# ru-wang/slam-plus-plus

Measured on AMD Instinct MI355X. Metric: Λ-solve block-nnz/sec + batch GN iters/sec, Venice BA, 1→8 MI355X, higher is better.
Workload: dtype f64; 1 GPU; venice871-shaped synthetic BA (871 cams, 530304 points, 2838740 observations, LM-damped); nnzb=3369915, n=1596138, mode=schur+dense, n_reduced=5226, schur_pairs=12875640, parallelism=single GPU

## Files before the change

### include/spp_hip.h

```cpp
#ifndef SPP_HIP_H
#define SPP_HIP_H

#include <stddef.h>
#include <stdint.h>

#ifdef __cplusplus
extern "C" {
#endif

#define SPP_OK            0
#define SPP_NOT_POSDEF    1
#define SPP_E_BADARG     -1
#define SPP_E_NOMEM      -2
#define SPP_E_HIP        -3
#define SPP_E_NO_DEVICE  -4
#define SPP_E_STATE      -5
#define SPP_E_UNSUPPORTED -6

#define SPP_MODE_AUTO     0
#define SPP_MODE_SPARSE   1
#define SPP_MODE_SCHUR    2
#define SPP_MODE_SCHUR_SPARSE 3

#define SPP_FLAG_PROFILE  1
// ... 153 lines not shown
#define SPP_PHASE_BACKSUBST 6
#define SPP_PHASE_ASSEMBLE  7
#define SPP_PHASE_TOTAL     8
#define SPP_N_PHASES        9
int spp_get_phase_ms(spp_ctx *ctx, double *ms_out );
int spp_get_dominant_kernel(spp_ctx *ctx, double *ms_total, int64_t *n_launches, double *flops);

int spp_microbench_copy(spp_ctx *ctx, size_t bytes, int iters, double *gb_per_s);
int spp_microbench_mfma_f64(spp_ctx *ctx, int iters, double *tflops);
int spp_microbench_ctile(spp_ctx *ctx, int n, int iters, double *gb_per_s);
int spp_microbench_update(spp_ctx *ctx, int64_t m, int iters, double *ms_per_launch);

int spp_dense_potrf_upper(spp_ctx *ctx, double *d_A, int64_t n, int64_t ld);
int spp_dense_posv(spp_ctx *ctx, double *d_A, int64_t n, int64_t ld, double *d_b);
int spp_dense_posv_masked(spp_ctx *ctx, double *d_A, int64_t n, int64_t ld, double *d_b, const uint64_t *words, int64_t nwords);
int spp_tile_mask_host(int64_t n, int bs, int64_t nblk, const int32_t *i1, const int32_t *i2, int has_rhs, int fill,
	uint64_t *words, int64_t *n_updates);
int spp_schur_tile_mask_host(int64_t nb, const int32_t *dim, const int64_t *col_ptr, const int64_t *row_idx, int shard_rank,
	int shard_world, uint64_t *words);
int spp_schur_cam_order_host(int64_t nb, const int32_t *dim, const int64_t *col_ptr, const int64_t *row_idx, int shard_rank,
	int shard_world, int flags, const int64_t *order_in, int64_t *cam_order, double *figures);
int spp_tail_order_host(int64_t n, int has_rhs, const uint64_t *words, int64_t nwords, int resident, int early, double beta,
	int32_t *table, int32_t *info);
int spp_dense_gemm_tn_sub(spp_ctx *ctx, int64_t m, int64_t n, int64_t k,
	const double *d_A, int64_t lda, const double *d_B, int64_t ldb, double *d_C, int64_t ldc);
int spp_dense_gemm_tn_sub_upper(spp_ctx *ctx, int64_t m, int64_t n, int64_t k,
	const double *d_A, int64_t lda, const double *d_B, int64_t ldb, double *d_C, int64_t ldc);
int spp_dense_front_factor(spp_ctx *ctx, double *d_F, int64_t ld, int64_t w, int64_t h, double *d_image);

const char *spp_version(void);

#ifdef __cplusplus
}
#endif
#endif
```

### slam_plus_plus_amd/api.py

```python
import ctypes
import os

import numpy as np

_HERE = os.path.dirname(os.path.abspath(__file__))
LIB_PATH = os.environ.get("SPP_LIB") or os.path.join(_HERE, "libspp_hip.so")

SPP_OK, SPP_NOT_POSDEF = 0, 1
MODE_AUTO, MODE_SPARSE, MODE_SCHUR, MODE_SCHUR_SPARSE, MODE_SCHUR_MIS = 0, 1, 2, 3, 4
FLAG_PROFILE = 1
INFO = dict(MODE=0, N=1, NNZB=2, NVALS=3, FACTOR_NNZ=4, FACTOR_FLOPS=5, N_REDUCED=6, N_POSES=7,
            N_LANDMARKS=8, SCHUR_PAIRS=9, N_OBS=10, SOLVE_BYTES=11, N_SUPERNODES=12, N_LEVELS=13, S_LD=14, S_NNZB=15, DENSE_STREAMED=16,
            LM_STREAM=17, BS_GROUPS=18, SCHUR_SIDE=19, S_CLEAR=20, S_DEVICE_PTR=21, ASM_HUB_CHUNK=22)
PHASES = ["permute", "schur_inv", "schur_gemm", "schur_rhs", "factor", "trisolve", "backsubst", "assemble", "total"]

EXPORTS = [
    "spp_create", "spp_destroy", "spp_free_memory", "spp_last_error", "spp_host_staging", "spp_set_stream", "spp_synchronize",
    "spp_analyze", "spp_set_shard", "spp_get_info", "spp_get_ordering", "spp_sparse_fronts", "spp_factor_solve",
    "spp_factor_solve_device", "spp_schur_buffer_size", "spp_schur_form", "spp_schur_finish",
    "spp_schur_packed_size", "spp_schur_pack", "spp_schur_unpack",
    "spp_assemble_analyze", "spp_assemble_get_structure", "spp_assemble_device", "spp_assemble_set_edge_weights",
    "spp_assemble_analyze_groups", "spp_assemble_groups_device", "spp_assemble_set_group_edge_weights",
    "spp_assemble_analyze_ternary", "spp_assemble_ternary_device", "spp_ba_intrinsics_linearize_device",
    "spp_ba_intrinsics_update_device",
    "spp_se2_linearize_at_device", "spp_se2_rb_linearize_device", "spp_slam2d_update_device",
    "spp_se3_linearize_at_device", "spp_se3_xyz_linearize_device", "spp_slam3d_update_device", "spp_rocv_range_linearize_device",
    "spp_rocv_cv_linearize_device", "spp_device_malloc",
    "spp_device_free", "spp_memcpy_h2d", "spp_memcpy_d2h", "spp_memcpy_d2d", "spp_get_phase_ms", "spp_get_dominant_kernel",
    "spp_microbench_copy", "spp_microbench_mfma_f64", "spp_microbench_ctile", "spp_microbench_update", "spp_block_ordering", "spp_schur_plan_host", "spp_set_profiling", "spp_se2_linearize_device", "spp_se2_update_device", "spp_ba_linearize_device", "spp_ba_stereo_linearize_device", "spp_ba_update_device", "spp_se3_linearize_device", "spp_se3_update_device", "spp_edge_chi2_device", "spp_edge_robust_weights_device", "spp_edge_hessian_maxdiag_device",
    "spp_lm_gain_denominator_device", "spp_dense_potrf_upper", "spp_dense_posv",
    "spp_dense_posv_masked", "spp_tile_mask_host", "spp_schur_tile_mask_host", "spp_tail_order_host", "spp_schur_cam_order_host",
    "spp_dense_gemm_tn_sub", "spp_dense_gemm_tn_sub_upper", "spp_dense_front_factor", "spp_version",
]

_lib = None
_c_i64p = ctypes.POINTER(ctypes.c_int64)
_c_i32p = ctypes.POINTER(ctypes.c_int32)
_c_f64p = ctypes.POINTER(ctypes.c_double)


class SppError(RuntimeError):
    """std::runtime_error of the C++ adapter (reference LinearSolver_Schur_GPU.cpp:734-797)."""


def load_library():
    global _lib
    if _lib is not None:
        return _lib
    if not os.path.exists(LIB_PATH):
        raise SppError("libspp_hip.so is not built: run `python -m slam_plus_plus_amd.build` "
                       "(hipcc --offload-arch=gfx950); there is no CPU fallback")
    lib = ctypes.CDLL(LIB_PATH)
    vp, i64, i32, dbl, cint = ctypes.c_void_p, ctypes.c_int64, ctypes.c_int32, ctypes.c_double, ctypes.c_int
    sig = {
# ... 47 lines not shown
        "spp_microbench_mfma_f64": (cint, [vp, cint, _c_f64p]),
        "spp_microbench_ctile": (cint, [vp, cint, cint, _c_f64p]),
        "spp_microbench_update": (cint, [vp, ctypes.c_int64, cint, _c_f64p]),
        "spp_block_ordering": (cint, [ctypes.c_int64, vp, vp, cint, vp]),
        "spp_schur_plan_host": (cint, [ctypes.c_int64, vp, vp, vp, cint, cint, cint, vp, vp]),
        "spp_set_profiling": (cint, [vp, cint]),
        "spp_se2_linearize_device": (cint, [vp, ctypes.c_int64, vp, vp, vp, vp, vp, vp, vp]),
        "spp_se2_update_device": (cint, [vp, ctypes.c_int64, vp, vp, cint, _c_f64p]),
        "spp_se3_linearize_device": (cint, [vp, ctypes.c_int64, vp, vp, vp, vp, vp, vp, vp]),
        "spp_se3_update_device": (cint, [vp, ctypes.c_int64, vp, vp, cint, _c_f64p]),
        "spp_edge_chi2_device": (cint, [vp, ctypes.c_int64, cint, vp, vp, _c_f64p]),
        "spp_edge_robust_weights_device": (cint, [vp, ctypes.c_int64, cint, cint, dbl, dbl, vp, vp]),
        "spp_edge_hessian_maxdiag_device": (cint, [vp, ctypes.c_int64, cint, cint, cint, vp, vp, vp, _c_f64p]),
        "spp_lm_gain_denominator_device": (cint, [vp, ctypes.c_int64, vp, vp, ctypes.c_double, _c_f64p]),
        "spp_ba_linearize_device": (cint, [vp, ctypes.c_int64, vp, vp, vp, vp, vp, vp, vp, vp, vp]),
        "spp_ba_stereo_linearize_device": (cint, [vp, ctypes.c_int64, vp, vp, vp, vp, vp, vp, vp, vp, vp]),
        "spp_ba_update_device": (cint, [vp, ctypes.c_int64, vp, vp, ctypes.c_int64, vp, vp, vp, ctypes.c_int64, cint, _c_f64p]),
        "spp_dense_potrf_upper": (cint, [vp, vp, i64, i64]),
        "spp_dense_posv": (cint, [vp, vp, i64, i64, vp]),
        "spp_dense_posv_masked": (cint, [vp, vp, i64, i64, vp, vp, i64]),
        "spp_tile_mask_host": (cint, [i64, cint, i64, vp, vp, cint, cint, vp, vp]),
        "spp_schur_tile_mask_host": (cint, [i64, vp, vp, vp, cint, cint, vp]),
        "spp_tail_order_host": (cint, [i64, cint, vp, i64, cint, cint, dbl, vp, vp]),
        "spp_schur_cam_order_host": (cint, [i64, vp, vp, vp, cint, cint, cint, vp, vp, vp]),
        "spp_dense_gemm_tn_sub": (cint, [vp, i64, i64, i64, vp, i64, vp, i64, vp, i64]),
        "spp_dense_gemm_tn_sub_upper": (cint, [vp, i64, i64, i64, vp, i64, vp, i64, vp, i64]),
        "spp_dense_front_factor": (cint, [vp, vp, i64, i64, i64, vp]),
        "spp_version": (ctypes.c_char_p, []),
    }
    for name, (res, args) in sig.items():
        fn = getattr(lib, name)
        fn.restype = res
        fn.argtypes = args
    _lib = lib
    return lib


def _ptr(a):
    return a.ctypes.data_as(ctypes.c_void_p)


ORDER_AMD, ORDER_ND = 0, 1


def block_ordering(lam, method=ORDER_AMD):
    lib = load_library()
# ... 56 lines not shown
    nc = int((dim == dim.max()).sum()) if not mis else int(dim.size)
    out = np.full(max(nc, 1), -1, dtype=np.int64)
    fig = np.zeros(8, dtype=np.float64)
    oin = None if order is None else np.ascontiguousarray(order, dtype=np.int64)
    if oin is not None and oin.size != nc:
        raise SppError("schur_cam_order_host: order must list every camera once")
    code = lib.spp_schur_cam_order_host(lam.nb, _ptr(dim), _ptr(col_ptr), _ptr(row_idx), shard_rank, shard_world,
                                        (1 if sparse_S else 0) | (2 if mis else 0),
                                        _ptr(oin) if oin is not None else None, _ptr(out), _ptr(fig))
    if code < 0:
        raise SppError("spp_schur_cam_order_host failed: %d" % code)
    keys = ("tiles", "updates", "path", "cost_us")
    natural = dict(zip(keys, (int(fig[0]), int(fig[1]), int(fig[2]), float(fig[3]))))
    chosen = dict(zip(keys, (int(fig[4]), int(fig[5]), int(fig[6]), float(fig[7]))))
    return out[out >= 0], bool(code), natural, chosen


def tail_order_host(n, words, has_rhs=True, resident=256, early=True, beta=0.0):
    lib = load_library()
    words = np.ascontiguousarray(words if words is not None else [], dtype=np.uint64)
    table = np.zeros(64 * 65 // 2 + 64, dtype=np.int32)
    info = np.zeros(5, dtype=np.int32)
    code = lib.spp_tail_order_host(int(n), 1 if has_rhs else 0, _ptr(words) if words.size else None, words.size, int(resident),
                                   1 if early else 0, float(beta), _ptr(table), _ptr(info))
    if code < 0:
        raise SppError("spp_tail_order_host failed: %d" % code)
    tiles = [(int(t) >> 16, int(t) & 0xffff) for t in table[:code]]
    return tiles, dict(zip(("n_early", "r_star", "rows_resident", "live_demand", "widest"), (int(v) for v in info)))


class DeviceArray:

    def __init__(self, ctx, n, dtype=np.float64):
        self.ctx, self.n, self.dtype = ctx, int(n), np.dtype(dtype)
        p = ctypes.c_void_p()
        ctx._check(ctx.lib.spp_device_malloc(ctx.h, self.n * self.dtype.itemsize, ctypes.byref(p)))
        self.ptr = p.value

    @classmethod
    def from_host(cls, ctx, arr):
        arr = np.ascontiguousarray(arr)
        d = cls(ctx, arr.size, arr.dtype)
        d.upload(arr)
        return d

    def upload(self, arr):
        arr = np.ascontiguousarray(arr, dtype=self.dtype)
        assert arr.size == self.n
        self.ctx._check(self.ctx.lib.spp_memcpy_h2d(self.ctx.h, self.ptr, _ptr(arr), arr.nbytes))

    def download(self):
# ... 347 lines not shown
```

### slam_plus_plus_amd/csrc/spp_api.cpp

```cpp

#include "spp_internal.h"
#include <string.h>
#include <new>

using namespace spp;

namespace spp {

void phases_reset(spp_ctx *ctx)
{
	if(!(ctx->flags & SPP_FLAG_PROFILE))
		return;
	if(!ctx->timer.created) {
		for(int i = 0; i < 2 * SPP_N_PHASES; ++ i)
			SPP_HIP_CHECK(hipEventCreate(&ctx->timer.ev[i]));
		ctx->timer.created = true;
	}
	for(int i = 0; i < SPP_N_PHASES; ++ i) {
		ctx->timer.used[i] = false;
		ctx->phase_ms[i] = 0;
	}
	ctx->dom_used = 0;
	ctx->dom_flops = 0;
}
// ... 1164 lines not shown
			*n_updates = upd;
		for(size_t q = 0; q < w.size(); ++ q)
			words[q] = w[q];
		return (int)w.size();
	} catch(...) {
		return SPP_E_NOMEM;
	}
}

int spp_tail_order_host(int64_t n, int has_rhs, const uint64_t *words, int64_t nwords, int resident, int early, double beta,
	int32_t *table, int32_t *info)
{
	const int64_t Tr = (n + DENSE_NB - 1) / DENSE_NB, Tc = has_rhs ? n / DENSE_NB + 1 : Tr;
	if(n <= 0 || Tr > 64 || Tc > 64 || nwords < 0 || (nwords && (!words || nwords != Tr)) || !table || !(beta >= 0))
		return SPP_E_BADARG;
	try {
		std::vector<uint64_t> bits((size_t)Tr + 1);
		const uint64_t all_cols = Tc == 64 ? ~0ull : (1ull << Tc) - 1;
		bits[0] = all_cols;
		for(int64_t i = 0; i < Tr; ++ i)
			bits[(size_t)i + 1] = (((nwords ? words[i] : all_cols) | (1ull << i)) & ~((1ull << i) - 1)) & all_cols;
		std::vector<int> order;
		int oinfo[5];
		const bool use = nwords && early;
		tail_order_table(bits, (int)Tr, (int)Tc, false, beta, use ? resident : 0, use, order, oinfo);
		for(size_t q = 0; q < order.size(); ++ q)
			table[q] = order[q];
		if(info)
			for(int q = 0; q < 5; ++ q)
				info[q] = oinfo[q];
		return (int)order.size();
	} catch(...) {
		return SPP_E_NOMEM;
	}
}

int spp_dense_posv_masked(spp_ctx *ctx, double *d_A, int64_t n, int64_t ld, double *d_b, const uint64_t *words, int64_t nwords)
{
	if(!ctx || !d_A || !d_b || n <= 0 || ld < n || nwords < 0 || (nwords && !words))
		return SPP_E_BADARG;
	SPP_TRY(ctx)
	SPP_HIP_CHECK(hipSetDevice(ctx->device));
	std::vector<uint64_t> mask(words, words + nwords);
	if(nwords) {
		SPP_REQUIRE(nwords == (n + DENSE_NB - 1) / DENSE_NB, SPP_E_BADARG, "posv: one mask word per tile row of 128");
		tile_mask_close(n, true, true, mask);
	}
	TileMaskGuard guard(ctx->dense, &mask);
	const int64_t ldp = ((n + 1 + DENSE_NB - 1) / DENSE_NB) * DENSE_NB;
	DevBuf<double> tmp;
	tmp.reserve((size_t)ldp * ldp);
	SPP_HIP_CHECK(hipMemsetAsync(tmp.p, 0, (size_t)ldp * ldp * sizeof(double), ctx->stream));
	SPP_HIP_CHECK(hipMemcpy2DAsync(tmp.p, ldp * sizeof(double), d_A, ld * sizeof(double), n * sizeof(double), n,
		hipMemcpyDeviceToDevice, ctx->stream));
// ... 55 lines not shown
```

### slam_plus_plus_amd/csrc/spp_dense.hip

```cpp

#include "spp_internal.h"
#include "spp_tiles.h"
#include "spp_dense_dev.h"
#include <stdio.h>
#include <stdlib.h>
#include <string.h>
#include <algorithm>
#include <vector>
#include <mutex>

namespace spp {


constexpr int BK = 16;
constexpr int LDS_STRIDE = 18;

template <int BM, int BN, int WM, int WN, int MODE, int DEPTH, int BKT, int SC1 = 0>
__device__ __forceinline__ void gemm_tn_tile(const int64_t m0, const int64_t n0, int64_t M, int64_t N, int K,
	const double *__restrict__ A, int64_t lda, const double *B, int64_t ldb, double *C, int64_t ldc, double *gemm_lds)
{
	constexpr int NWM = BM / WM, NWN = BN / WN, NT = NWM * NWN * 64;
	constexpr int TA = WM / 16, TB = WN / 16;
	constexpr int PPC = BKT / 2, LSTR = BKT + 2;
	constexpr int PA = (BM * PPC) / NT, PB = (BN * PPC) / NT;
// ... 1257 lines not shown
	for(int i = -1; i < Tr; ++ i) {
		const int64_t g = k + 1 + i;
		uint64_t w = (mask && g >= 0) ? ((*mask)[(size_t)g] >> (k + 1)) : all_cols;
		if(i >= 0)
			w = (w | (1ull << i)) & ~((1ull << i) - 1);
		bits[(size_t)i + 1] = w & all_cols;
	}
	hipStream_t s = ctx->stream;
	static uint64_t attr_seen = 0;
	if(first_on_this_device(attr_seen))
		SPP_HIP_CHECK(hipFuncSetAttribute((const void*)dense_tail_kernel, hipFuncAttributeMaxDynamicSharedMemorySize,
			TAIL_LDS_DOUBLES * (int)sizeof(double)));
	if(dw.tail_pub.cap < (size_t)Tr * Tc) {
		dw.tail_pub.reserve(std::max<size_t>((size_t)Tr * Tc, 24 * 25));
		SPP_HIP_CHECK(hipMemsetAsync(dw.tail_pub.p, 0, dw.tail_pub.cap * sizeof(int), s));
		dw.tail_epoch = 0;
	}
	if(dw.tail_dinv.cap < (size_t)Tr * 8 * 256)
		dw.tail_dinv.reserve(std::max<size_t>((size_t)Tr * 8 * 256, (size_t)24 * 8 * 256));
	if(++ dw.tail_epoch >= (1 << 26)) {
		SPP_HIP_CHECK(hipMemsetAsync(dw.tail_pub.p, 0, dw.tail_pub.cap * sizeof(int), s));
		dw.tail_epoch = 1;
	}
	const bool early = mask != nullptr && sw.tail_early != 0;
	if(early && dw.tail_resident < 0) {
		int per_cu = 0;
		hipDeviceProp_t prop;
		if(hipOccupancyMaxActiveBlocksPerMultiprocessor(&per_cu, (const void*)dense_tail_kernel, POTRF_THREADS,
		   TAIL_LDS_DOUBLES * sizeof(double)) == hipSuccess && hipGetDeviceProperties(&prop, ctx->device) == hipSuccess)
			dw.tail_resident = std::max(per_cu, 0) * prop.multiProcessorCount;
		else {
			(void)hipGetLastError();
			dw.tail_resident = 0;
		}
	}
	if(dw.tail_order_tr != Tr || dw.tail_order_tc != Tc || dw.tail_order_bits != bits || dw.tail_order_pre != (k >= 0) ||
	   dw.tail_order_masked != early) {
		if(!dw.tail_order_host.empty())
			SPP_HIP_CHECK(hipStreamSynchronize(s));
		std::vector<int> &order = dw.tail_order_host;
		int oinfo[5];
		tail_order_table(bits, Tr, Tc, k >= 0, sw.tail_order_beta, early ? dw.tail_resident : 0, early, order, oinfo);
		if(sw.verbose)
			fprintf(stderr, "[spp] streamed tail: %d x %d tiles, %d listed, %d resident; %d tiles of rows %d.. seated first (whole rows resident %d, live demand %d)\n",
				Tr, Tc, (int)order.size(), early ? dw.tail_resident : 0, oinfo[0], oinfo[1], oinfo[2], oinfo[3]);
		dw.tail_order.upload(order, s);
		dw.tail_order_tr = Tr;
		dw.tail_order_tc = Tc;
		dw.tail_order_bits = bits;
		dw.tail_order_pre = k >= 0;
		dw.tail_order_masked = early;
	}
	const int ntile = (int)dw.tail_order_host.size();
	TailArgs a;
	a.order = dw.tail_order.p;
	memset(a.rowbits, 0, sizeof(a.rowbits));
	for(size_t q = 0; q < bits.size(); ++ q)
		a.rowbits[q] = bits[q];
	a.A = d_A;
	a.ld = ld;
	a.rows = rows;
	a.ncols = ncols;
	a.c0 = c1;
	a.have_pre = (k >= 0) ? 1 : 0;
	a.Tr = Tr;
	a.Tc = Tc;
// ... 610 lines not shown
```

### slam_plus_plus_amd/csrc/spp_internal.h

```cpp
#pragma once

#include <hip/hip_runtime.h>
#include <stdint.h>
#include <string>
#include <vector>
#include <sys/mman.h>
#include <utility>
#include <new>
#include <exception>
#include <thread>
#include <stdexcept>
#include <algorithm>
#include <string.h>
#include <chrono>
#include <stdio.h>
#include <stdlib.h>
#include "../../include/spp_hip.h"
#include "spp_switches.h"

namespace spp {

struct Error : std::runtime_error {
	int code;
	Error(int c, const std::string &what) : std::runtime_error(what), code(c) {}
// ... 206 lines not shown
	DevBuf<double> xw;
	DevBuf<double> partial;
	DevBuf<double> S;
	bool unlisted_dirty = true;
	bool side_pending = false, side_padded = false;
	int side_last = 0, clear_last = 0;
	void release_all();
};

struct DenseWork {
	DevBuf<double> tinv;
	DevBuf<int> info;
	DevBuf<double> tinv_all;
	int64_t tinv_half = 0;
	DevBuf<double> xtmp;
	DevBuf<int> flags;
	DevBuf<int> tail_pub;
	DevBuf<double> tail_dinv;
	int tail_epoch = 0;
	DevBuf<int> tail_order;
	std::vector<int> tail_order_host;
	int tail_order_tr = 0, tail_order_tc = 0;
	std::vector<uint64_t> tail_order_bits;
	bool tail_order_pre = false, tail_order_masked = false;
	int tail_resident = -1;
	const std::vector<uint64_t> *tile_mask = nullptr;
	bool tail_masked_whole = false;
	int tail_rows_last = 0;
	bool tail_disabled = false;
	DevBuf<double> trsv_m;
	DevBuf<double> trsv_pay;
	uint64_t epoch = 0;
	int *h_chain_err = nullptr;
	hipStream_t aux = nullptr;
	hipEvent_t ev[2] = {nullptr, nullptr};
	DevBuf<int> sync;
	DevBuf<int> fuse_cnt;
	std::vector<int> fuse_expect;
	bool fuse_dirty = false;
	int64_t ident_from = -1;
	hipStream_t chain = nullptr;
	hipEvent_t ev_chain = nullptr;
	DevBuf<int> la_cnt;
	DevBuf<long long> la_trace;
	int la_state = 0;
	int la_reserve = 0;
	int la_ncu = 0;
// ... 70 lines not shown
	const double *d_Om);
double lm_gain_denominator(spp_ctx *ctx, int64_t n, const double *d_dx, const double *d_rhs, double alpha);
void se3_linearize(spp_ctx *ctx, int64_t ne, const int32_t *d_v0, const int32_t *d_v1, const double *d_poses,
	const double *d_meas, double *d_J0, double *d_J1, double *d_r);
double se3_update(spp_ctx *ctx, int64_t nv, double *d_poses, const double *d_dx, bool apply);
void ba_linearize(spp_ctx *ctx, int64_t no, const int32_t *d_cam_of, const int32_t *d_pt_of, const double *d_cams,
	const double *d_intr, const double *d_pts, const double *d_meas, double *d_J0, double *d_J1, double *d_r);
void ba_stereo_linearize(spp_ctx *ctx, int64_t no, const int32_t *d_cam_of, const int32_t *d_pt_of, const double *d_cams,
	const double *d_intr, const double *d_pts, const double *d_meas, double *d_J0, double *d_J1, double *d_r);
void ba_intrinsics_linearize(spp_ctx *ctx, int64_t no, const int32_t *d_cam_of, const int32_t *d_pt_of, const int32_t *d_intr_of,
	const double *d_cams, const double *d_intr, const double *d_pts, const double *d_meas, double *d_J0, double *d_J1, double *d_J2,
	double *d_r);
double ba_intrinsics_update(spp_ctx *ctx, int64_t ni, double *d_intr, const int64_t *d_intr_dxoff, const double *d_dx, bool apply);
double ba_update(spp_ctx *ctx, int64_t nc, double *d_cams, const int64_t *d_cam_dxoff, int64_t np, double *d_pts,
	const int64_t *d_pt_dxoff, const double *d_dx, int64_t n_dx, bool apply);

void min_degree_order(int64_t nb, const int64_t *col_ptr, const int64_t *row_idx, std::vector<int64_t> &order);
void nested_dissection_order(int64_t nb, const int64_t *col_ptr, const int64_t *row_idx, std::vector<int64_t> &order);

void tile_mask_mark(int64_t n, int bs, int64_t nblk, const int32_t *i1, const int32_t *i2, std::vector<uint64_t> &words);
int64_t tile_mask_close(int64_t n, bool has_rhs, bool fill, std::vector<uint64_t> &words);
constexpr double TAIL_MODEL_STEP_US = 36.5, TAIL_MODEL_UPDATE_US = 2.0, TAIL_MODEL_START_US = 45.0;
constexpr int TAIL_MODEL_RESIDENT = 256;
struct TileDagCost {
	int64_t tiles = 0, updates = 0, path = 0;
	double cost_us = 0;
};
TileDagCost tile_dag_cost(int64_t n, const std::vector<uint64_t> &filled, int resident);
void tail_order_table(const std::vector<uint64_t> &bits, int Tr, int Tc, bool have_pre, double beta, int resident, bool early,
	std::vector<int> &order, int *info);

void build_schur_plan(spp_ctx *ctx, bool sparse_S, bool mis = false);
int64_t schur_buffer_doubles(const spp_ctx *ctx);
bool schur_applicable(const Structure &st, int *dp, int *dl);
double schur_plan_host_probe(const Structure &st, int shard_rank, int shard_world, bool sparse_S, bool mis, int64_t *out);
void schur_tile_mask_host_probe(const Structure &st, std::vector<uint64_t> &words);
bool schur_cam_order_host_probe(const Structure &st, int shard_rank, int shard_world, bool sparse_S, bool mis, const int64_t *order_in,
	std::vector<int32_t> &cam_order, TileDagCost cost[2]);

void sparse_analyze(spp_ctx *ctx, const Structure &st);
int sparse_factor_solve(spp_ctx *ctx, const double *d_vals, double *d_rhs);
void sparse_release(spp_ctx *ctx);
void sparse_dag_disable(spp_ctx *ctx);
int64_t sparse_info(const spp_ctx *ctx, int what);
int64_t sparse_fronts(const spp_ctx *ctx, int64_t capacity, int32_t *h, int32_t *w, int32_t *pad, int32_t *cls, int32_t *level,
	int32_t *parent, int32_t *team);

constexpr int64_t SCHUR_SIDE_MIN_OBS = 500000;
void schur_form(spp_ctx *ctx, const double *d_vals, const double *d_rhs, double *d_S_rhs, bool one_call = false);
int schur_finish(spp_ctx *ctx, const double *d_vals, double *d_S_rhs, double *d_rhs);
void schur_pack(spp_ctx *ctx, double *S, double *packed, bool pack);

constexpr int DENSE_NB = 128;
// ... 99 lines not shown
```

### slam_plus_plus_amd/csrc/spp_schur_plan.cpp

```cpp

#include "spp_internal.h"
#include <sys/mman.h>
#include <stdlib.h>
#include <algorithm>
#include <numeric>
#include <string.h>
#include <stdio.h>
#include <thread>
#include <memory>
#include <chrono>
#include <exception>

namespace spp {

void SchurPlan::release_all()
{
	lm_ptr.release(); bs_ptr.release(); n_bs = 0; lm_coff.release(); lm_rbase.release(); obs_pose.release(); obs_lm.release();
	obs_off.release(); pose_rbase.release(); cam_ptr.release(); cam_obs.release(); items.release();
	obs_wpos.release(); xcd_beg.release(); sblk_i1.release(); sblk_i2.release(); sblk_aoff.release();
	sblk_voff.release(); s_st = Structure(); sparse_S = false; mis = false;
	pair_a.release(); pair_b.release(); multi_blk.release(); multi_ptr.release(); cinv.release(); lfac.release();
	W.release(); Up.release(); xw.release(); partial.release(); S.release();
	pose_block.clear(); lm_block.clear(); is_lm.clear(); tile_mask.clear();
}
// ... 226 lines not shown
		uint64_t cols = 0;
		const uint64_t *r = g.row(c);
		for(int64_t w = 0; w < g.nw; ++ w)
			for(uint64_t m = r[w]; m; m &= m - 1)
				cols |= tl[w * 64 + __builtin_ctzll(m)];
		for(uint64_t rows = tl[c]; rows; rows &= rows - 1) {
			const int a = __builtin_ctzll(rows);
			if(a < Tr)
				words[a] |= cols;
		}
	}
	tile_mask_close(n_red, true, true, words);
}

static bool cam_order_live_ok(const std::vector<uint64_t> &filled, int64_t n_red)
{
	const int Tr = (int)filled.size(), Tc = (int)(n_red / DENSE_NB + 1);
	std::vector<uint64_t> bits((size_t)Tr + 1);
	bits[0] = Tc == 64 ? ~0ull : (1ull << Tc) - 1;
	for(int i = 0; i < Tr; ++ i)
		bits[(size_t)i + 1] = filled[i];
	std::vector<int> order;
	int info[5];
	tail_order_table(bits, Tr, Tc, false, 0.0, TAIL_MODEL_RESIDENT, true, order, info);
	return info[0] > 0 || info[3] <= TAIL_MODEL_RESIDENT;
}

static bool cam_dissect(const CamGraph &g, int dp, int64_t n_red, std::vector<int32_t> &order, TileDagCost cost[2])
{
	const int64_t nc = g.nc, nw = g.nw;
	order.resize((size_t)nc);
	std::vector<int32_t> pos((size_t)nc);
	for(int64_t c = 0; c < nc; ++ c)
		order[c] = pos[c] = (int32_t)c;
	std::vector<uint64_t> words;
	cam_graph_mask(g, pos, dp, n_red, words);
	if(words.empty())
		return false;
	cost[0] = cost[1] = tile_dag_cost(n_red, words, TAIL_MODEL_RESIDENT);
	int64_t al = DENSE_NB;
	for(int64_t x = dp, y = DENSE_NB; y; ) {
		const int64_t t = x % y;
		x = y;
		y = t;
		if(!y)
			al = DENSE_NB / x;
	}
// ... 1040 lines not shown
```

### slam_plus_plus_amd/csrc/spp_switches.h

```cpp
#pragma once

#include <stdint.h>
#include <stdlib.h>
#include <string.h>
#include <algorithm>

namespace spp {

constexpr long long WAIT_TICKS_PER_MS = 100000;
constexpr long long WAIT_TICKS_DEFAULT = 500 * WAIT_TICKS_PER_MS;

enum Ordering { ORDERING_AUTO, ORDERING_AMD, ORDERING_ND };
constexpr int MID_FRONT_MAX = 640;

struct Switches {
	bool verbose;
	int plan_threads;
	int64_t plan_min_work;

	int dense_sched;
	int fused;
	int aux_reserve_cus;
	int tile_444;
	int dense_la;
// ... 56 lines not shown
}

inline Switches parse_switches()
{
	Switches w;
	w.verbose = getenv("SPP_VERBOSE") != nullptr;
	const char *threads = getenv("SPP_PLAN_THREADS");
	w.plan_threads = threads ? std::max(1, atoi(threads)) : 0;
	w.plan_min_work = std::max<int64_t>(1, env_i64("SPP_PLAN_MIN_WORK", int64_t(1) << 18));

	w.dense_sched = env_int("SPP_DENSE_SCHED", 1);
	w.fused = env_int("SPP_FUSED", 1);
	w.aux_reserve_cus = env_int("SPP_AUX_RESERVE_CUS", 32);
	w.tile_444 = env_int("SPP_TILE_444", 0);
	w.dense_la = env_int("SPP_DENSE_LA", 0);
	w.la_chain_mask = env_int("SPP_LA_CHAIN_MASK", 1);
	w.la_g2 = env_int("SPP_LA_G2", 0);
	w.la_bulk_acquire = env_int("SPP_LA_BULK_ACQUIRE", 1);
	w.la_slots = env_i64("SPP_LA_SLOTS", 0);
	w.la_trace = env_int("SPP_LA_TRACE", 0);
	w.tail_rows = env_int("SPP_DENSE_TAIL", 1) ? env_int("SPP_TAIL_ROWS", 44) : 0;
	w.tail_mask = env_int("SPP_TAIL_MASK", 1);
	w.tail_order_beta = env_double("SPP_TAIL_ORDER_BETA", 0.0);
	w.tail_early = env_int("SPP_TAIL_EARLY", 1);
	w.tail_timeout_ticks = env_i64("SPP_TAIL_TIMEOUT_TICKS", WAIT_TICKS_DEFAULT);
	w.tail_trace = env_int("SPP_TAIL_TRACE", 0);
	w.trsv_chain = env_int("SPP_TRSV_CHAIN", 2);
	w.trsv_mform = env_int("SPP_TRSV_MFORM", 1);

	w.sacc_ulm = env_int("SPP_SACC_ULM", 1) != 0;
	w.sacc_factored = env_int("SPP_SACC_FACTORED", 1) != 0;
	w.sacc_tile = std::max<int64_t>(1, env_i64("SPP_SACC_TILE", 4));
	w.sacc_tile_cols = env_i64("SPP_SACC_TILE_COLS", -2);
	w.sacc_xcd = env_int("SPP_SACC_XCD", 1);
	w.sacc_chunk = env_int("SPP_SACC_CHUNK", 1);
	w.schur_cam_order = env_int("SPP_SCHUR_CAM_ORDER", 1);
	w.backsubst_fused = env_int("SPP_BACKSUBST_FUSED", 1);
	w.schur_side = env_int("SPP_SCHUR_SIDE", 1);
	w.lm_stream = env_int("SPP_LM_STREAM", 1);

	w.mid_front_max = std::max(128, std::min(MID_FRONT_MAX, env_int("SPP_MID_FRONT_MAX", 320)));
	const char *ordering = getenv("SPP_ORDERING");
	w.ordering = !ordering ? ORDERING_AUTO : (!strcmp(ordering, "nd") ? ORDERING_ND : ORDERING_AMD);
	w.amalg_small = env_i64("SPP_AMALG_SMALL", 32);
	w.amalg_zeros = env_double("SPP_AMALG_ZEROS", 0.12);
	w.amalg_relax_h = env_i64("SPP_AMALG_RELAX_H", 96);
	w.amalg_zeros_small = env_double("SPP_AMALG_ZEROS_SMALL", 0.2);
// ... 18 lines not shown
```

### slam_plus_plus_amd/csrc/spp_tile_plan.cpp

```cpp

#include "spp_internal.h"
#include <algorithm>

namespace spp {

void tile_mask_mark(int64_t n, int bs, int64_t nblk, const int32_t *i1, const int32_t *i2, std::vector<uint64_t> &words)
{
	words.clear();
	const int64_t Tr = (n + DENSE_NB - 1) / DENSE_NB, Tc = n / DENSE_NB + 1;
	if(Tr < 1 || Tc > 64)
		return;
	words.assign((size_t)Tr, 0);
	for(int64_t q = 0; q < nblk; ++ q) {
		const int64_t a = std::min(i1[q], i2[q]), b = std::max(i1[q], i2[q]);
		const int64_t r0 = a * bs / DENSE_NB, r1 = std::min<int64_t>(a * bs + bs - 1, n - 1) / DENSE_NB;
		const int64_t c0 = b * bs / DENSE_NB, c1 = std::min<int64_t>(b * bs + bs - 1, n - 1) / DENSE_NB;
		if(a < 0 || r0 >= Tr || c0 >= Tr)
			continue;
		words[r0] |= (1ull << c0) | (1ull << c1);
		words[r1] |= (1ull << c0) | (1ull << c1);
	}
}

int64_t tile_mask_close(int64_t n, bool has_rhs, bool fill, std::vector<uint64_t> &words)
{
// ... 5 lines not shown
	const uint64_t cols = Tc == 64 ? ~0ull : (1ull << Tc) - 1;
	for(int64_t i = 0; i < Tr; ++ i) {
		words[i] |= 1ull << i;
		if(has_rhs)
			words[i] |= 1ull << (n / DENSE_NB);
		words[i] &= cols & ~((1ull << i) - 1);
	}
	int64_t updates = 0;
	for(int64_t k = 0; k < Tr; ++ k) {
		const uint64_t r = words[k] & ~((2ull << k) - 1);
		for(uint64_t m = r; m; m &= m - 1) {
			const int a = __builtin_ctzll(m);
			if(a >= Tr)
				break;
			const uint64_t f = r & ~((1ull << a) - 1);
			if(fill)
				words[a] |= f;
			updates += __builtin_popcountll(words[a] & f);
		}
	}
	return updates;
}

void tail_order_table(const std::vector<uint64_t> &bits, int Tr, int Tc, bool have_pre, double beta, int resident, bool early,
	std::vector<int> &order, int *info)
{
	std::vector<std::pair<double, int> > key;
	for(int i = 0; i < Tr; ++ i)
		for(int j = i; j < Tc; ++ j)
			if((bits[(size_t)i + 1] >> j) & 1)
				key.push_back(std::make_pair((double)i + beta * (double)j, (i << 16) | j));
	std::stable_sort(key.begin(), key.end(), [](const std::pair<double, int> &x, const std::pair<double, int> &y) { return x.first < y.first; });
	order.resize(key.size());
	for(size_t q = 0; q < key.size(); ++ q)
		order[q] = key[q].second;
	int widest = 1;
	for(int i = 0; i < Tr; ++ i)
		widest = std::max(widest, (int)__builtin_popcountll(bits[(size_t)i + 1]));
	const int D = std::max(resident, 0) / widest;
	if(info) {
		info[0] = 0;
		info[1] = Tr;
		info[2] = D;
		info[3] = 0;
		info[4] = widest;
	}
	if(!early || resident <= 0)
// ... 23 lines not shown
		if(i >= r_star)
			++ n_early;
		else {
			++ live[(size_t)std::max(first_step(i, j), 0)];
			-- live[(size_t)i + 1];
		}
	}
	int demand = 0;
	for(int r = 0, run = 0; r < Tr; ++ r) {
		run += live[(size_t)r];
		demand = std::max(demand, run);
	}
	if(info)
		info[3] = demand;
	if(n_early == 0 || n_early > resident / 2 || resident - n_early < demand)
		return;
	std::stable_partition(order.begin(), order.end(), [r_star](const int t) { return (t >> 16) >= r_star; });
	if(info) {
		info[0] = n_early;
		info[1] = r_star;
	}
}

TileDagCost tile_dag_cost(int64_t n, const std::vector<uint64_t> &filled, int resident)
{
	TileDagCost c;
	const int64_t Tr = (int64_t)filled.size();
	std::vector<uint64_t> w(filled);
	c.updates = tile_mask_close(n, true, true, w);
	std::vector<int> depth((size_t)Tr, 1);
	for(int64_t k = 0; k < Tr; ++ k) {
		c.tiles += __builtin_popcountll(w[k]);
		for(int64_t j = 0; j < k; ++ j)
			if((w[j] >> k) & 1)
				depth[k] = std::max(depth[k], depth[j] + 1);
		c.path = std::max<int64_t>(c.path, depth[k]);
	}
	c.cost_us = std::max(c.path * TAIL_MODEL_STEP_US, c.updates * TAIL_MODEL_UPDATE_US / std::max(1, resident)) + TAIL_MODEL_START_US;
	return c;
}

}
```

Measured before the change: 1.306 billion block-nnz/s.

## Order streamed dense-tail tiles by simulated deadlines instead of row heuristic

Adds a host-side discrete-event model of the streamed dense Cholesky tail, in which tiles are seated into a fixed number of resident slots and wait on producer panels. A new early-seating mode (default 2) uses the model to pick which tiles to seat first by a latest-start threshold, keeping an order only if it is predicted clearly better and does not stall with one fewer slot. The goal is to shorten the tail's critical path by seating late-critical tiles early. It adds host planning time per table build and depends on hand-tuned model constants matching the GPU.

```diff
diff --git a/include/spp_hip.h b/include/spp_hip.h
--- a/include/spp_hip.h
+++ b/include/spp_hip.h
@@ -199,6 +199,8 @@
 	int shard_world, int flags, const int64_t *order_in, int64_t *cam_order, double *figures);
 int spp_tail_order_host(int64_t n, int has_rhs, const uint64_t *words, int64_t nwords, int resident, int early, double beta,
 	int32_t *table, int32_t *info);
+int spp_tail_sim_host(int64_t n, int has_rhs, const uint64_t *words, int64_t nwords, int resident, const int32_t *table, int64_t ntable,
+	double *row_times, double *figures);
 int spp_dense_gemm_tn_sub(spp_ctx *ctx, int64_t m, int64_t n, int64_t k,
 	const double *d_A, int64_t lda, const double *d_B, int64_t ldb, double *d_C, int64_t ldc);
 int spp_dense_gemm_tn_sub_upper(spp_ctx *ctx, int64_t m, int64_t n, int64_t k,
diff --git a/slam_plus_plus_amd/api.py b/slam_plus_plus_amd/api.py
--- a/slam_plus_plus_amd/api.py
+++ b/slam_plus_plus_amd/api.py
@@ -29,7 +29,7 @@
     "spp_device_free", "spp_memcpy_h2d", "spp_memcpy_d2h", "spp_memcpy_d2d", "spp_get_phase_ms", "spp_get_dominant_kernel",
     "spp_microbench_copy", "spp_microbench_mfma_f64", "spp_microbench_ctile", "spp_microbench_update", "spp_block_ordering", "spp_schur_plan_host", "spp_set_profiling", "spp_se2_linearize_device", "spp_se2_update_device", "spp_ba_linearize_device", "spp_ba_stereo_linearize_device", "spp_ba_update_device", "spp_se3_linearize_device", "spp_se3_update_device", "spp_edge_chi2_device", "spp_edge_robust_weights_device", "spp_edge_hessian_maxdiag_device",
     "spp_lm_gain_denominator_device", "spp_dense_potrf_upper", "spp_dense_posv",
-    "spp_dense_posv_masked", "spp_tile_mask_host", "spp_schur_tile_mask_host", "spp_tail_order_host", "spp_schur_cam_order_host",
+    "spp_dense_posv_masked", "spp_tile_mask_host", "spp_schur_tile_mask_host", "spp_tail_order_host", "spp_tail_sim_host", "spp_schur_cam_order_host",
     "spp_dense_gemm_tn_sub", "spp_dense_gemm_tn_sub_upper", "spp_dense_front_factor", "spp_version",
 ]
 
@@ -123,6 +123,7 @@
         "spp_tile_mask_host": (cint, [i64, cint, i64, vp, vp, cint, cint, vp, vp]),
         "spp_schur_tile_mask_host": (cint, [i64, vp, vp, vp, cint, cint, vp]),
         "spp_tail_order_host": (cint, [i64, cint, vp, i64, cint, cint, dbl, vp, vp]),
+        "spp_tail_sim_host": (cint, [i64, cint, vp, i64, cint, vp, i64, vp, vp]),
         "spp_schur_cam_order_host": (cint, [i64, vp, vp, vp, cint, cint, cint, vp, vp, vp]),
         "spp_dense_gemm_tn_sub": (cint, [vp, i64, i64, i64, vp, i64, vp, i64, vp, i64]),
         "spp_dense_gemm_tn_sub_upper": (cint, [vp, i64, i64, i64, vp, i64, vp, i64, vp, i64]),
@@ -225,11 +226,33 @@
     table = np.zeros(64 * 65 // 2 + 64, dtype=np.int32)
     info = np.zeros(5, dtype=np.int32)
     code = lib.spp_tail_order_host(int(n), 1 if has_rhs else 0, _ptr(words) if words.size else None, words.size, int(resident),
-                                   1 if early else 0, float(beta), _ptr(table), _ptr(info))
+                                   _early_value(early), float(beta), _ptr(table), _ptr(info))
     if code < 0:
         raise SppError("spp_tail_order_host failed: %d" % code)
     tiles = [(int(t) >> 16, int(t) & 0xffff) for t in table[:code]]
     return tiles, dict(zip(("n_early", "r_star", "rows_resident", "live_demand", "widest"), (int(v) for v in info)))
+
+
+def _early_value(early):
+    if isinstance(early, (bool, np.bool_)):
+        return 1 if early else 0
+    if int(early) not in (0, 1, 2):
+        raise SppError("tail_order_host: early is 0, 1 or 2")
+    return int(early)
+
+
+def tail_sim_host(n, words, tiles, has_rhs=True, resident=256):
+    lib = load_library()
+    words = np.ascontiguousarray(words if words is not None else [], dtype=np.uint64)
+    table = np.ascontiguousarray([(i << 16) | j for i, j in tiles], dtype=np.int32)
+    Tr = -(-int(n) // 128)
+    rows = np.zeros(3 * max(Tr, 1), dtype=np.float64)
+    fig = np.zeros(2, dtype=np.float64)
+    code = lib.spp_tail_sim_host(int(n), 1 if has_rhs else 0, _ptr(words) if words.size else None, words.size, int(resident),
+                                 _ptr(table), table.size, _ptr(rows), _ptr(fig))
+    if code < 0:
+        raise SppError("spp_tail_sim_host failed: %d" % code)
+    return dict(makespan=float(fig[0]), stalled=bool(fig[1]), rows=[tuple(float(v) for v in rows[3 * i:3 * i + 3]) for i in range(code)])
 
 
 class DeviceArray:
diff --git a/slam_plus_plus_amd/csrc/spp_api.cpp b/slam_plus_plus_amd/csrc/spp_api.cpp
--- a/slam_plus_plus_amd/csrc/spp_api.cpp
+++ b/slam_plus_plus_amd/csrc/spp_api.cpp
@@ -1210,7 +1210,7 @@
 			bits[(size_t)i + 1] = (((nwords ? words[i] : all_cols) | (1ull << i)) & ~((1ull << i) - 1)) & all_cols;
 		std::vector<int> order;
 		int oinfo[5];
-		const bool use = nwords && early;
+		const int use = nwords ? early : 0;
 		tail_order_table(bits, (int)Tr, (int)Tc, false, beta, use ? resident : 0, use, order, oinfo);
 		for(size_t q = 0; q < order.size(); ++ q)
 			table[q] = order[q];
@@ -1218,6 +1218,44 @@
 			for(int q = 0; q < 5; ++ q)
 				info[q] = oinfo[q];
 		return (int)order.size();
+	} catch(...) {
+		return SPP_E_NOMEM;
+	}
+}
+
+int spp_tail_sim_host(int64_t n, int has_rhs, const uint64_t *words, int64_t nwords, int resident, const int32_t *table, int64_t ntable,
+	double *row_times, double *figures)
+{
+	const int64_t Tr = (n + DENSE_NB - 1) / DENSE_NB, Tc = has_rhs ? n / DENSE_NB + 1 : Tr;
+	if(n <= 0 || Tr > 64 || Tc > 64 || nwords < 0 || (nwords && (!words || nwords != Tr)) || !table || ntable < 0 || !figures)
+		return SPP_E_BADARG;
+	try {
+		std::vector<uint64_t> bits((size_t)Tr + 1);
+		const uint64_t all_cols = Tc == 64 ? ~0ull : (1ull << Tc) - 1;
+		bits[0] = all_cols;
+		for(int64_t i = 0; i < Tr; ++ i)
+			bits[(size_t)i + 1] = (((nwords ? words[i] : all_cols) | (1ull << i)) & ~((1ull << i) - 1)) & all_cols;
+		std::vector<uint64_t> seen((size_t)Tr, 0);
+		int64_t listed = 0;
+		for(int64_t i = 0; i < Tr; ++ i)
+			listed += __builtin_popcountll(bits[(size_t)i + 1]);
+		if(ntable != listed)
+			return SPP_E_BADARG;
+		std::vector<int> order((size_t)ntable);
+		for(int64_t q = 0; q < ntable; ++ q) {
+			const int i = table[q] >> 16, j = table[q] & 0xffff;
+			if(table[q] < 0 || i >= Tr || j >= Tc || !((bits[(size_t)i + 1] >> j) & 1) || ((seen[(size_t)i] >> j) & 1))
+				return SPP_E_BADARG;
+			seen[(size_t)i] |= 1ull << j;
+			order[(size_t)q] = table[q];
+		}
+		const TailSeatSim sim = tail_seat_sim(bits, (int)Tr, (int)Tc, false, order, resident);
+		figures[0] = sim.makespan;
+		figures[1] = sim.stalled ? 1.0 : 0.0;
+		if(row_times)
+			for(size_t q = 0; q < sim.rows.size(); ++ q)
+				row_times[q] = sim.rows[q];
+		return (int)Tr;
 	} catch(...) {
 		return SPP_E_NOMEM;
 	}
diff --git a/slam_plus_plus_amd/csrc/spp_dense.hip b/slam_plus_plus_amd/csrc/spp_dense.hip
--- a/slam_plus_plus_amd/csrc/spp_dense.hip
+++ b/slam_plus_plus_amd/csrc/spp_dense.hip
@@ -1303,7 +1303,7 @@
 		SPP_HIP_CHECK(hipMemsetAsync(dw.tail_pub.p, 0, dw.tail_pub.cap * sizeof(int), s));
 		dw.tail_epoch = 1;
 	}
-	const bool early = mask != nullptr && sw.tail_early != 0;
+	const int early = mask != nullptr ? sw.tail_early : 0;
 	if(early && dw.tail_resident < 0) {
 		int per_cu = 0;
 		hipDeviceProp_t prop;
@@ -1321,8 +1321,18 @@
 			SPP_HIP_CHECK(hipStreamSynchronize(s));
 		std::vector<int> &order = dw.tail_order_host;
 		int oinfo[5];
-		tail_order_table(bits, Tr, Tc, k >= 0, sw.tail_order_beta, early ? dw.tail_resident : 0, early, order, oinfo);
-		if(sw.verbose)
+		double deadline[3];
+		const std::chrono::steady_clock::time_point t_table = std::chrono::steady_clock::now();
+		tail_order_table(bits, Tr, Tc, k >= 0, sw.tail_order_beta, early ? dw.tail_resident : 0, early, order, oinfo, deadline);
+		if(sw.verbose && early == 2) {
+			uint32_t sum = 2166136261u;
+			for(size_t q = 0; q < order.size(); ++ q)
+				for(int b = 0; b < 4; ++ b)
+					sum = (sum ^ (((uint32_t)order[q] >> (8 * b)) & 255u)) * 16777619u;
+			fprintf(stderr, "[spp] streamed tail by deadline: %d x %d tiles, %d listed, %d resident; |E| = %d tiles from row %d on, theta %.3f us, simulated %.3f us against %.3f us of SPP_TAIL_EARLY=1; table %08x, built in %.2f ms\n",
+				Tr, Tc, (int)order.size(), dw.tail_resident, oinfo[0], oinfo[1], deadline[0], deadline[1], deadline[2], sum,
+				std::chrono::duration<double>(std::chrono::steady_clock::now() - t_table).count() * 1e3);
+		} else if(sw.verbose)
 			fprintf(stderr, "[spp] streamed tail: %d x %d tiles, %d listed, %d resident; %d tiles of rows %d.. seated first (whole rows resident %d, live demand %d)\n",
 				Tr, Tc, (int)order.size(), early ? dw.tail_resident : 0, oinfo[0], oinfo[1], oinfo[2], oinfo[3]);
 		dw.tail_order.upload(order, s);
diff --git a/slam_plus_plus_amd/csrc/spp_internal.h b/slam_plus_plus_amd/csrc/spp_internal.h
--- a/slam_plus_plus_amd/csrc/spp_internal.h
+++ b/slam_plus_plus_amd/csrc/spp_internal.h
@@ -252,7 +252,8 @@
 	std::vector<int> tail_order_host;
 	int tail_order_tr = 0, tail_order_tc = 0;
 	std::vector<uint64_t> tail_order_bits;
-	bool tail_order_pre = false, tail_order_masked = false;
+	bool tail_order_pre = false;
+	int tail_order_masked = 0;
 	int tail_resident = -1;
 	const std::vector<uint64_t> *tile_mask = nullptr;
 	bool tail_masked_whole = false;
@@ -369,13 +370,20 @@
 int64_t tile_mask_close(int64_t n, bool has_rhs, bool fill, std::vector<uint64_t> &words);
 constexpr double TAIL_MODEL_STEP_US = 36.5, TAIL_MODEL_UPDATE_US = 2.0, TAIL_MODEL_START_US = 45.0;
 constexpr int TAIL_MODEL_RESIDENT = 256;
+constexpr double TAIL_MODEL_CATCHUP_US = 2.6, TAIL_MODEL_PANEL_US = 31.5, TAIL_MODEL_HANDOVER_US = 0.7, TAIL_MODEL_LOAD_US = 11.0;
 struct TileDagCost {
 	int64_t tiles = 0, updates = 0, path = 0;
 	double cost_us = 0;
 };
 TileDagCost tile_dag_cost(int64_t n, const std::vector<uint64_t> &filled, int resident);
-void tail_order_table(const std::vector<uint64_t> &bits, int Tr, int Tc, bool have_pre, double beta, int resident, bool early,
-	std::vector<int> &order, int *info);
+void tail_order_table(const std::vector<uint64_t> &bits, int Tr, int Tc, bool have_pre, double beta, int resident, int early,
+	std::vector<int> &order, int *info, double *deadline = nullptr);
+struct TailSeatSim {
+	double makespan = 0;
+	bool stalled = false;
+	std::vector<double> rows;
+};
+TailSeatSim tail_seat_sim(const std::vector<uint64_t> &bits, int Tr, int Tc, bool have_pre, const std::vector<int> &order, int resident);
 
 void build_schur_plan(spp_ctx *ctx, bool sparse_S, bool mis = false);
 int64_t schur_buffer_doubles(const spp_ctx *ctx);
diff --git a/slam_plus_plus_amd/csrc/spp_schur_plan.cpp b/slam_plus_plus_amd/csrc/spp_schur_plan.cpp
--- a/slam_plus_plus_amd/csrc/spp_schur_plan.cpp
+++ b/slam_plus_plus_amd/csrc/spp_schur_plan.cpp
@@ -272,7 +272,7 @@
 		bits[(size_t)i + 1] = filled[i];
 	std::vector<int> order;
 	int info[5];
-	tail_order_table(bits, Tr, Tc, false, 0.0, TAIL_MODEL_RESIDENT, true, order, info);
+	tail_order_table(bits, Tr, Tc, false, 0.0, TAIL_MODEL_RESIDENT, 1, order, info);
 	return info[0] > 0 || info[3] <= TAIL_MODEL_RESIDENT;
 }
 
diff --git a/slam_plus_plus_amd/csrc/spp_switches.h b/slam_plus_plus_amd/csrc/spp_switches.h
--- a/slam_plus_plus_amd/csrc/spp_switches.h
+++ b/slam_plus_plus_amd/csrc/spp_switches.h
@@ -102,7 +102,7 @@
 	w.tail_rows = env_int("SPP_DENSE_TAIL", 1) ? env_int("SPP_TAIL_ROWS", 44) : 0;
 	w.tail_mask = env_int("SPP_TAIL_MASK", 1);
 	w.tail_order_beta = env_double("SPP_TAIL_ORDER_BETA", 0.0);
-	w.tail_early = env_int("SPP_TAIL_EARLY", 1);
+	w.tail_early = env_int("SPP_TAIL_EARLY", 2);
 	w.tail_timeout_ticks = env_i64("SPP_TAIL_TIMEOUT_TICKS", WAIT_TICKS_DEFAULT);
 	w.tail_trace = env_int("SPP_TAIL_TRACE", 0);
 	w.trsv_chain = env_int("SPP_TRSV_CHAIN", 2);
diff --git a/slam_plus_plus_amd/csrc/spp_tile_plan.cpp b/slam_plus_plus_amd/csrc/spp_tile_plan.cpp
--- a/slam_plus_plus_amd/csrc/spp_tile_plan.cpp
+++ b/slam_plus_plus_amd/csrc/spp_tile_plan.cpp
@@ -1,6 +1,7 @@
 
 #include "spp_internal.h"
 #include <algorithm>
+#include <functional>
 
 namespace spp {
 
@@ -52,7 +53,7 @@
 	return updates;
 }
 
-void tail_order_table(const std::vector<uint64_t> &bits, int Tr, int Tc, bool have_pre, double beta, int resident, bool early,
+static void tail_order_rows(const std::vector<uint64_t> &bits, int Tr, int Tc, bool have_pre, double beta, int resident, bool early,
 	std::vector<int> &order, int *info)
 {
 	std::vector<std::pair<double, int> > key;
@@ -122,6 +123,275 @@
 	}
 }
 
+namespace {
+
+struct TailSim {
+	int Tr, Tc, kfirst;
+	const std::vector<uint64_t> &bits;
+	std::vector<int> steps_off, steps;
+	std::vector<int> cons_off, cons;
+	std::vector<int> n_prod;
+	std::vector<double> pub, seat;
+	std::vector<int> missing, ready;
+	std::vector<double> heap;
+
+	TailSim(const std::vector<uint64_t> &b, int tr, int tc, bool have_pre)
+		:Tr(tr), Tc(tc), kfirst(have_pre ? -1 : 0), bits(b)
+	{
+		const size_t nt = (size_t)Tr * Tc;
+		steps_off.assign(nt + 1, 0);
+		n_prod.assign(nt, 0);
+		std::vector<int> n_cons(nt, 0);
+		for(int pass = 0; pass < 2; ++ pass) {
+			if(pass) {
+				cons_off.assign(nt + 1, 0);
+				for(size_t t = 0; t < nt; ++ t)
+					cons_off[t + 1] = cons_off[t] + n_cons[t];
+				cons.resize((size_t)cons_off[nt]);
+				steps.resize((size_t)steps_off[nt]);
+				std::fill(n_cons.begin(), n_cons.end(), 0);
+			}
+			for(int i = 0; i < Tr; ++ i) {
+				for(int j = i; j < Tc; ++ j) {
+					if(!listed(i, j))
+						continue;
+					const int t = i * Tc + j;
+					int ns = 0;
+					for(int k = kfirst; k < i; ++ k) {
+						const uint64_t w = bits[(size_t)k + 1];
+						if(!((w >> i) & (w >> j) & 1))
+							continue;
+						if(pass)
+							steps[(size_t)steps_off[t] + ns] = k;
+						++ ns;
+						if(k < 0)
+							continue;
+						const int pa = k * Tc + i, pb = k * Tc + j;
+						if(pass) {
+							cons[(size_t)cons_off[pa] + n_cons[pa]] = t;
+							if(pb != pa)
+								cons[(size_t)cons_off[pb] + n_cons[pb]] = t;
+						} else
+							n_prod[t] += (pb != pa) ? 2 : 1;
+						++ n_cons[pa];
+						if(pb != pa)
+							++ n_cons[pb];
+					}
+					if(j != i) {
+						const int pd = i * Tc + i;
+						if(pass)
+							cons[(size_t)cons_off[pd] + n_cons[pd]] = t;
+						else
+							++ n_prod[t];
+						++ n_cons[pd];
+					}
+					if(!pass)
+						steps_off[t + 1] = ns;
+				}
+			}
+			if(!pass)
+				for(size_t t = 0; t < nt; ++ t)
+					steps_off[t + 1] += steps_off[t];
+		}
+	}
+
+	bool listed(const int i, const int j) const { return (bits[(size_t)i + 1] >> j) & 1; }
+	int n_steps(const int i, const int j) const { return steps_off[(size_t)i * Tc + j + 1] - steps_off[(size_t)i * Tc + j]; }
+
+	double run_tile(const int t, TailSeatSim &out)
+	{
+		const int i = t / Tc, j = t % Tc;
+		double at = seat[t] + TAIL_MODEL_LOAD_US;
+		const double behind = (i == j) ? TAIL_MODEL_UPDATE_US : TAIL_MODEL_CATCHUP_US;
+		for(int q = steps_off[t]; q < steps_off[t + 1]; ++ q) {
+			const int k = steps[q];
+			if(k < 0) {
+				for(int J = 0; J < 8; ++ J)
+					at += behind;
+				continue;
+			}
+			const double *pa = &pub[(size_t)(k * Tc + i) * 8], *pb = &pub[(size_t)(k * Tc + j) * 8];
+			if(std::max(pa[7], pb[7]) + TAIL_MODEL_HANDOVER_US <= at) {
+				for(int J = 0; J < 8; ++ J)
+					at += behind;
+				continue;
+			}
+			for(int J = 0; J < 8; ++ J) {
+				const double r = std::max(pa[J], pb[J]) + TAIL_MODEL_HANDOVER_US;
+				at = (r > at) ? r + TAIL_MODEL_UPDATE_US : at + behind;
+			}
+		}
+		double *mine = &pub[(size_t)t * 8];
+		if(i == j) {
+			for(int J = 0; J < 8; ++ J)
+				mine[J] = at + (J + 1) * (TAIL_MODEL_PANEL_US / 8);
+			out.rows[3 * (size_t)i] = seat[t];
+			out.rows[3 * (size_t)i + 1] = at;
+			out.rows[3 * (size_t)i + 2] = mine[7];
+		} else {
+			const double *pd = &pub[(size_t)(i * Tc + i) * 8];
+			for(int J = 0; J < 8; ++ J) {
+				const double r = pd[J] + TAIL_MODEL_HANDOVER_US;
+				at = (r > at) ? r + TAIL_MODEL_UPDATE_US : at + TAIL_MODEL_CATCHUP_US;
+				mine[J] = at;
+			}
+		}
+		return mine[7];
+	}
+
+	void run(const std::vector<int> &order, const int resident, TailSeatSim &out)
+	{
+		const size_t nt = (size_t)Tr * Tc, n = order.size();
+		pub.assign(nt * 8, 0.0);
+		seat.assign(nt, -1.0);
+		missing = n_prod;
+		ready.clear();
+		heap.clear();
+		out.makespan = 0;
+		out.stalled = false;
+		out.rows.assign(3 * (size_t)Tr, 0.0);
+		size_t next = 0, done = 0;
+		auto seat_next = [&](const double at) {
+			const int t = (order[next] >> 16) * Tc + (order[next] & 0xffff);
+			seat[t] = at;
+			if(missing[t] == 0)
+				ready.push_back(t);
+			++ next;
+		};
+		while(next < n && next < (size_t)std::max(resident, 0))
+			seat_next(0.0);
+		for(;;) {
+			while(!ready.empty()) {
+				const int t = ready.back();
+				ready.pop_back();
+				const double fin = run_tile(t, out);
+				++ done;
+				out.makespan = std::max(out.makespan, fin);
+				heap.push_back(fin);
+				std::push_heap(heap.begin(), heap.end(), std::greater<double>());
+				for(int q = cons_off[t]; q < cons_off[t + 1]; ++ q) {
+					const int c = cons[q];
+					if(-- missing[c] == 0 && seat[c] >= 0)
+						ready.push_back(c);
+				}
+			}
+			if(next == n)
+				break;
+			if(heap.empty()) {
+				out.stalled = true;
+				return;
+			}
+			std::pop_heap(heap.begin(), heap.end(), std::greater<double>());
+			const double at = heap.back();
+			heap.pop_back();
+			seat_next(at);
+		}
+		out.stalled = done < n;
+	}
+};
+
+}
+
+TailSeatSim tail_seat_sim(const std::vector<uint64_t> &bits, int Tr, int Tc, bool have_pre, const std::vector<int> &order, int resident)
+{
+	TailSim sim(bits, Tr, Tc, have_pre);
+	TailSeatSim out;
+	sim.run(order, resident, out);
+	return out;
+}
+
+static void tail_order_deadline(const std::vector<uint64_t> &bits, int Tr, int Tc, bool have_pre, double beta, int resident,
+	std::vector<int> &order, int *info, double *deadline)
+{
+	const int D = info[2];
+	std::vector<int> base;
+	tail_order_rows(bits, Tr, Tc, have_pre, beta, resident, false, base, nullptr);
+	TailSim sim(bits, Tr, Tc, have_pre);
+	TailSeatSim s1, s;
+	sim.run(order, resident, s1);
+	if(deadline) {
+		deadline[0] = 0;
+		deadline[1] = deadline[2] = s1.makespan;
+	}
+	if(s1.stalled)
+		return;
+	std::vector<int> depth((size_t)Tr, 1);
+	for(int k = 0; k < Tr; ++ k)
+		for(int j = 0; j < k; ++ j)
+			if((bits[(size_t)j + 1] >> k) & 1)
+				depth[k] = std::max(depth[k], depth[j] + 1);
+	struct Cand { double ls; int pos, tile; };
+	std::vector<Cand> cand;
+	std::vector<double> all_ls;
+	for(size_t q = 0; q < base.size(); ++ q) {
+		const int i = base[q] >> 16, j = base[q] & 0xffff;
+		const double ls = (depth[i] - 1) * TAIL_MODEL_STEP_US - 8 * TAIL_MODEL_CATCHUP_US * sim.n_steps(i, j);
+		all_ls.push_back(ls);
+		if(i >= D && sim.seat[(size_t)i * Tc + j] > ls)
+			cand.push_back(Cand{ls, (int)q, base[q]});
+	}
+	std::sort(all_ls.begin(), all_ls.end());
+	all_ls.erase(std::unique(all_ls.begin(), all_ls.end()), all_ls.end());
+	std::sort(cand.begin(), cand.end(), [](const Cand &x, const Cand &y) { return x.ls < y.ls || (x.ls == y.ls && x.pos < y.pos); });
+	std::vector<int> table, best;
+	std::vector<char> in_e(base.size());
+	double best_ms = 0, best_theta = 0;
+	size_t best_ne = 0, ne = 0, seen = 0;
+	for(size_t th = 0; th < all_ls.size(); ++ th) {
+		while(ne < cand.size() && cand[ne].ls < all_ls[th])
+			++ ne;
+		if(ne > (size_t)resident / 2)
+			break;
+		if(ne == seen)
+			continue;
+		seen = ne;
+		table.clear();
+		std::fill(in_e.begin(), in_e.end(), 0);
+		for(size_t q = 0; q < ne; ++ q) {
+			table.push_back(cand[q].tile);
+			in_e[(size_t)cand[q].pos] = 1;
+		}
+		for(size_t q = 0; q < base.size(); ++ q)
+			if(!in_e[q])
+				table.push_back(base[q]);
+		sim.run(table, resident, s);
+		if(!s.stalled && (best.empty() || s.makespan < best_ms)) {
+			best = table;
+			best_ms = s.makespan;
+			best_theta = all_ls[th];
+			best_ne = ne;
+		}
+	}
+	if(best.empty() || !(best_ms <= 0.98 * s1.makespan))
+		return;
+	sim.run(best, resident - 1, s);
+	if(s.stalled)
+		return;
+	order = best;
+	int r_min = Tr;
+	for(size_t q = 0; q < best_ne; ++ q)
+		r_min = std::min(r_min, best[q] >> 16);
+	info[0] = (int)best_ne;
+	info[1] = r_min;
+	if(deadline) {
+		deadline[0] = best_theta;
+		deadline[1] = best_ms;
+	}
+}
+
+void tail_order_table(const std::vector<uint64_t> &bits, int Tr, int Tc, bool have_pre, double beta, int resident, int early,
+	std::vector<int> &order, int *info, double *deadline)
+{
+	int oinfo[5];
+	tail_order_rows(bits, Tr, Tc, have_pre, beta, resident, early != 0, order, oinfo);
+	if(deadline)
+		deadline[0] = deadline[1] = deadline[2] = 0;
+	if(early == 2 && resident > 0)
+		tail_order_deadline(bits, Tr, Tc, have_pre, beta, resident, order, oinfo, deadline);
+	if(info)
+		std::copy(oinfo, oinfo + 5, info);
+}
+
 TileDagCost tile_dag_cost(int64_t n, const std::vector<uint64_t> &filled, int resident)
 {
 	TileDagCost c;
```

After: 1.319 billion block-nnz/s (median of 5 runs). 1.01x the previous value.
